# MECLabTUDA/Lifelong-nnUNet

Hardware: AMD Instinct MI355X
Metric: 3D patches/sec (whole node) + mean Dice vs ref, 5-level 3D Generic_UNet training step (higher is better)
Workload: dtype f16 (fp32 accumulate, fp32 master weights); 1 GPU; BASELINE configs[1]: nnUNetTrainerSequential.run_iteration, 160x192x160 patches, batch 2/GPU, num_pool 5, base 32, 3 logits; global_batch=2, parallelism=dp1, distinct_resident_batches=2, deterministic_wgrad=False

## Files before the change

### include/lnn_hip.h

```cpp
#ifndef LNN_HIP_H
#define LNN_HIP_H

#include <stddef.h>
#include <stdint.h>

#ifdef __cplusplus
extern "C" {
#endif

typedef void* lnn_stream_t;

enum lnn_status {
    LNN_OK = 0,
    LNN_ERR_BAD_ARG = -1,
    LNN_ERR_WORKSPACE = -2,
    LNN_ERR_LAUNCH = -3,
    LNN_ERR_UNSUPPORTED = -4
};

const char* lnn_last_error(void);
int lnn_version(void);
int lnn_device_info(int* cu_count, int* clock_khz, char* name, int name_len);

int lnn_pack_weights(lnn_stream_t s, const float* src, void* dst_h, int ntaps, int M, int KC,
// ... 60 lines not shown
int lnn_instnorm_lrelu_seg_bwd(lnn_stream_t s, void* y_inout_h, const void* dz_prior_h, int ld_dz, const float* seg_w,
                               const float* dlogits, float* seg_dw, int K, int N, long V, int C, const float* mean,
                               const float* rstd, const float* gamma, const float* beta, float slope, float* dgamma,
                               float* dbeta, float grad_unscale, double* ws);
size_t lnn_instnorm_lrelu_seg_bwd_ws_doubles(int N, int C);
int lnn_instnorm_lrelu_bwd_sums(lnn_stream_t s, const void* y_h, const void* dz_h, int ld_dz, int N, long V, int C,
                                const float* mean, const float* rstd, const float* gamma, const float* beta, float slope,
                                float* dgamma, float* dbeta, float grad_unscale, double* ws);
int lnn_conv3d_wgrad_c1_in_bwd(lnn_stream_t s, const void* x_h, const void* y_h, const void* dz_h, int ld_dz, float* dwp, int N,
                               int D, int H, int W, int K, const float* mean, const float* rstd, const float* gamma,
                               const float* beta, float slope, const double* ws, float* parts, long parts_elems);
int lnn_conv3d_dgrad_in_bwd_sums(lnn_stream_t s, const void* dy, int ld_dy, const void* wp, void* dx, int ld_dx, int N, int Di,
                                 int Hi, int Wi, int C, int K, const void* u_h, const float* mean, const float* rstd,
                                 const float* gamma, const float* beta, float slope, float* dgamma, float* dbeta,
                                 float grad_unscale, double* ws, float* splitk_ws, long splitk_elems);
int lnn_instnorm_lrelu_bwd_apply(lnn_stream_t s, void* y_h, const void* dz_h, int ld_dz, int N, long V, int C, const float* mean,
                                 const float* rstd, const float* gamma, const float* beta, float slope, double* ws);
int lnn_instnorm_small_volume(void);
int lnn_conv3d_fwd_in_lrelu(lnn_stream_t s, const void* x_a, const void* x_b, int ld_x, int c_a, const void* wp, const float* bias,
                            void* y, int N, int Di, int Hi, int Wi, int C, int K, int stride, float eps, float* mean, float* rstd,
                            const float* gamma, const float* beta, float slope, void* z_h, int ld_z, double* ws, float* splitk_ws,
                            long splitk_elems);
int lnn_conv3d_dgrad_in_bwd(lnn_stream_t s, const void* dy, int ld_dy, const void* wp, void* dx, int ld_dx, int N, int Di, int Hi,
                            int Wi, int C, int K, void* u_h, const float* mean, const float* rstd, const float* gamma,
                            const float* beta, float slope, float* dgamma, float* dbeta, float grad_unscale, double* ws,
                            float* splitk_ws, long splitk_elems);

int lnn_seg1x1_fwd(lnn_stream_t s, const void* z_h, int ld_z, const float* w, float* logits, int N, long V,
                   int C, int K);
int lnn_seg1x1_bwd(lnn_stream_t s, const void* z_h, int ld_z, const float* w, const float* dlogits, void* dz_h,
// ... 117 lines not shown
```

### lifelong-nnunet_amd/csrc/igemm_common.h

```cpp
#pragma once
#include "lnn_common.h"

struct TapTable {
    int ntaps;
    int taps_per_group;
    unsigned short pos_off[27];
    unsigned char slot[27];
};

struct ConvParams {
    const half_t* x;
    const half_t* x2;
    half_t* y2;
    int csplit = 0x7fffffff, msplit = 0x7fffffff;
    const half_t* wp;
    const float* bias;
    half_t* y;
    int ld_x, ld_y;
    int N, Di, Hi, Wi, Do, Ho, Wo;
    int C, M, Mpad, KCpad;
    int wtaps;
    int Ld, Lh, Lw;
    int tiles_z, tiles_y, tiles_x;
    int os, par_z, par_y, par_x;
// ... 28 lines not shown
                            const float* beta, float slope, float* mean, float* rstd);
int lnn_launch_in_small_bwd(hipStream_t s, void* y, const void* dz, int ld_dz, int N, long V, int C, const float* mean, const float* rstd,
                            const float* gamma, const float* beta, float slope, double* ws, float* dgamma, float* dbeta, float unscale);
int lnn_launch_in_stats_finalize(hipStream_t s, const float* pws, int nslots, int N, int C, long V, float eps, float* mean, float* rstd);
int lnn_launch_in_bwd_sums_raw(hipStream_t s, const float* pws, int nslots, int N, int C, const float* mean, const float* rstd,
                               double* ws, float* dgamma, float* dbeta, float unscale);
int lnn_launch_conv_s1_v9(hipStream_t s, ConvParams& p, const char* name);
int lnn_conv_k133_on_v9(hipStream_t s, const void* x, int ld_x, const void* wp, const float* bias, void* y, int ld_y, int N, int D, int H,
                        int W, int C, int M, int flip, const char* name);
bool lnn_conv_s1_mt_supported(const ConvParams& p);
double lnn_conv_s1_mt_efficiency(const ConvParams& p);
int lnn_conv_s1_mt_ksplit(const ConvParams& p, const float* ws, long ws_elems);
int lnn_launch_conv_s1_mt(hipStream_t s, ConvParams& p, float* ws, long ws_elems, const char* name);
int lnn_launch_up2_dgrad(hipStream_t s, ConvParams& p, const char* name);
int lnn_launch_up2_convT(hipStream_t s, ConvParams& p, const char* name);
int lnn_launch_down2_conv(hipStream_t s, ConvParams& p, const char* name);
int lnn_launch_down2_convT_dgrad(hipStream_t s, ConvParams& p, const char* name);
bool lnn_down2s_supported(const ConvParams& p);
int lnn_down2s_stats_slots(const ConvParams& p);
int lnn_launch_down2s(hipStream_t s, ConvParams& p, const char* name);
```

### lifelong-nnunet_amd/csrc/igemm_conv.hip

```cpp
#include "lnn_common.h"
#include "igemm_common.h"
#include "igemm_gen.h"
#include <cstdlib>

namespace {

typedef unsigned c1_uint4 __attribute__((ext_vector_type(4)));

template <bool STATS>
__global__ __launch_bounds__(256, 3) void conv_c1_fwd_kernel(const ConvParams p, int tiles_per_sample) {
    constexpr int TZ = 4, TY = 8, TX = 8, VT = TZ * TY * TX / 128, PZ = TZ + 2, PY = TY + 2, PX = TX + 2, P = PZ * PY * PX;
    constexpr int NL = (P + 255) / 256;
    __shared__ half_t xl[P];
    __shared__ float sred[STATS ? 4 * 2 * 32 : 1];
    const int tid = threadIdx.x, lane = tid & 63, wave = tid >> 6;
    const int n = blockIdx.y;
    const int m0 = blockIdx.z * 32;
    const long xbase_n = (long)n * p.Di * p.Hi * p.Wi;
    const int v = lane & 31, hk = lane >> 5;
    half8 a[2];
#pragma unroll
    for (int k16 = 0; k16 < 2; ++k16) a[k16] = *reinterpret_cast<const half8*>(p.wp + lnn_panel_off(0, m0 + v, k16 * 16 + hk * 8, 1, 32));
    int toff[2][8];
#pragma unroll
// ... 373 lines not shown
}
}

extern "C" int lnn_conv3d_dgrad(lnn_stream_t s, const void* dy, int ld_dy, const void* wp, void* dx, int ld_dx, int N,
                                int Di, int Hi, int Wi, int C, int K, int stride, int accumulate) {
    return conv3d_dgrad_impl(s, dy, ld_dy, wp, dx, nullptr, 0, ld_dx, N, Di, Hi, Wi, C, K, stride, accumulate);
}

extern "C" int lnn_conv3d_dgrad_ws(lnn_stream_t s, const void* dy, int ld_dy, const void* wp, void* dx, int ld_dx, int N, int Di, int Hi,
                                   int Wi, int C, int K, int stride, int accumulate, float* splitk_ws, long splitk_elems) {
    return conv3d_dgrad_impl(s, dy, ld_dy, wp, dx, nullptr, 0, ld_dx, N, Di, Hi, Wi, C, K, stride, accumulate, splitk_ws, splitk_elems);
}

static int g_last_dgrad_reduce_fused = 0;
extern "C" int lnn_debug_last_dgrad_reduce_fused(void) { return g_last_dgrad_reduce_fused; }

extern "C" int lnn_conv3d_dgrad_in_bwd_sums(lnn_stream_t s_, const void* dy, int ld_dy, const void* wp, void* dx, int ld_dx, int N,
                                            int Di, int Hi, int Wi, int C, int K, const void* u, const float* mean, const float* rstd,
                                            const float* gamma, const float* beta, float slope, float* dgamma, float* dbeta,
                                            float grad_unscale, double* ws, float* splitk_ws, long splitk_elems) {
    hipStream_t s = (hipStream_t)s_;
    LNN_REQUIRE(u && lnn_aligned16(u) && mean && rstd && gamma && beta && ws, "lnn_conv3d_dgrad_in_bwd_sums: null / misaligned parameter");
    const long V = (long)Di * Hi * Wi;
    ConvParams p{};
    p.x = (const half_t*)dy; p.y = (half_t*)dx; p.ld_x = ld_dy; p.ld_y = ld_dx; p.N = N;
    p.Di = Di; p.Hi = Hi; p.Wi = Wi; p.Do = Di; p.Ho = Hi; p.Wo = Wi; p.C = K; p.M = C; p.os = 1;
    p.Ld = Di; p.Lh = Hi; p.Lw = Wi; p.pad_lo = 1;
    p.red_ld = C;
    static int no_fuse = -1;
    if (no_fuse < 0) { const char* e = getenv("LNN_NO_FUSED_IN_BWD_REDUCE"); no_fuse = (e && e[0] == '1') ? 1 : 0; }
    const bool fused = !no_fuse && wp && dx && dy && lnn_aligned16(dx) && lnn_aligned16(dy) && use_v9(p) && lnn_conv_s1_v9_red_supported(p) &&
                       !lnn_gen_prefers(LNN_GEN_OP_CONV_S1, (long)N * V);
    g_last_dgrad_reduce_fused = fused ? 1 : 0;
    if (!fused) {
        if (int e = conv3d_dgrad_impl(s_, dy, ld_dy, wp, dx, nullptr, 0, ld_dx, N, Di, Hi, Wi, C, K, 1, 0, splitk_ws, splitk_elems)) return e;
        return lnn_instnorm_lrelu_bwd_sums(s_, u, dx, ld_dx, N, V, C, mean, rstd, gamma, beta, slope, dgamma, dbeta, grad_unscale, ws);
    }
    LNN_REQUIRE(lnn_aligned16(wp), "lnn_conv3d_dgrad_in_bwd_sums: weight panel misaligned");
    if (int e = check_act(dy, ld_dy, K, "lnn_conv3d_dgrad_in_bwd_sums(dy)")) return e;
    if (int e = check_act(dx, ld_dx, C, "lnn_conv3d_dgrad_in_bwd_sums(dx)")) return e;
    p.wp = (const half_t*)wp; p.bias = nullptr;
    p.Mpad = lnn_round_up(C, 32); p.KCpad = lnn_round_up(K, 16); p.wtaps = 27;
    p.taps.ntaps = 27;
    for (int t = 0; t < 27; ++t) {
        const int dz = t / 9, dyy = (t / 3) % 3, dxx = t % 3;
        p.taps.pos_off[t] = (unsigned short)((dz * 10 + dyy) * 10 + dxx);
        p.taps.slot[t] = (unsigned char)((2 - dz) * 9 + (2 - dyy) * 3 + (2 - dxx));
    }
    p.dbg = g_dbg;
    float* pws = reinterpret_cast<float*>(ws + (size_t)N * C * 3);
    p.stats_pws = pws;
    p.red_u = (const half_t*)u; p.red_mean = mean; p.red_rstd = rstd; p.red_gamma = gamma; p.red_beta = beta; p.red_slope = slope;
    if (int e = lnn_launch_conv_s1_v9(s, p, "lnn_conv3d_dgrad_in_bwd_sums(s1,v9,reduce)")) return e;
    return lnn_launch_in_bwd_sums_raw(s, pws, p.stats_nblk, N, C, mean, rstd, ws, dgamma, dbeta, grad_unscale);
}

extern "C" int lnn_conv3d_dgrad_in_bwd(lnn_stream_t s_, const void* dy, int ld_dy, const void* wp, void* dx, int ld_dx, int N, int Di,
                                       int Hi, int Wi, int C, int K, void* u, const float* mean, const float* rstd, const float* gamma,
                                       const float* beta, float slope, float* dgamma, float* dbeta, float grad_unscale, double* ws,
                                       float* splitk_ws, long splitk_elems) {
    LNN_REQUIRE(u && lnn_aligned16(u) && mean && rstd && gamma && beta && ws, "lnn_conv3d_dgrad_in_bwd: null / misaligned parameter");
    const long V = (long)Di * Hi * Wi;
    LNN_REQUIRE(V <= lnn_instnorm_small_volume(), "lnn_conv3d_dgrad_in_bwd: %ld voxels per sample (limit %d): use lnn_conv3d_dgrad_in_bwd_sums",
                V, lnn_instnorm_small_volume());
    LNN_REQUIRE(C % 8 == 0, "lnn_conv3d_dgrad_in_bwd: %d channels (multiple of 8)", C);
    if (int rc = conv3d_dgrad_impl(s_, dy, ld_dy, wp, dx, nullptr, 0, ld_dx, N, Di, Hi, Wi, C, K, 1, 0, splitk_ws, splitk_elems)) return rc;
    return lnn_launch_in_small_bwd((hipStream_t)s_, u, dx, ld_dx, N, V, C, mean, rstd, gamma, beta, slope, ws, dgamma, dbeta, grad_unscale);
}

// ... 74 lines not shown
```

### lifelong-nnunet_amd/csrc/igemm_up2.hip

```cpp
#include "igemm_common.h"

namespace {

constexpr int TZ = 2, TY = 8, TX = 8, PZ = 3, PY = 9, PX = 9;
constexpr int P = PZ * PY * PX;
constexpr int CK = 16, ROWB = 32, MB = 32;
constexpr int XBYTES = P * ROWB;
constexpr int XCHUNKS = P * 2;
constexpr int NT = 256;
constexpr int XN = (XCHUNKS + NT - 1) / NT;

template <int MODE>
struct UpCfg {
    static constexpr int NTAP = MODE == 0 ? 27 : 8;
    static constexpr int WBYTES = NTAP * MB * ROWB;
    static constexpr int WCHUNKS = NTAP * MB * 2;
    static constexpr int WN = (WCHUNKS + NT - 1) / NT;
};

__device__ __forceinline__ int up_xaddr(int pz, int py, int px, int c2) {
    return ((pz * PY + py) * PX + px) * ROWB + ((c2 ^ (py & 1)) << 4);
}
__device__ __forceinline__ int up_waddr(int row, int c2) { return row * ROWB + ((c2 ^ ((row >> 3) & 1)) << 4); }

__device__ __forceinline__ void up_lane_voxel(int v, int& r, int& x) {
    if (v < 4) { r = 0; x = v; }
    else if (v < 12) { r = 2; x = v - 4; }
    else if (v < 16) { r = 0; x = v - 8; }
    else if (v < 20) { r = 3; x = v - 16; }
    else if (v < 28) { r = 1; x = v - 20; }
    else { r = 3; x = v - 24; }
}

template <int MODE>
__global__ __launch_bounds__(NT, 2) void igemm_up2_kernel(const ConvParams p, int mblocks) {
    using Cfg = UpCfg<MODE>;
    constexpr int WN = Cfg::WN, WBYTES = Cfg::WBYTES, WCHUNKS = Cfg::WCHUNKS;
    extern __shared__ __attribute__((aligned(16))) char smem[];
    char* const xb = smem;
    char* const wb = smem + 2 * XBYTES;

    const int tid = threadIdx.x, lane = tid & 63, wave = tid >> 6;
    const int v = lane & 31, hk = lane >> 5;
    const int m0 = (blockIdx.x % mblocks) * MB;
    int t = blockIdx.x / mblocks;
    const int tx = t % p.tiles_x; t /= p.tiles_x;
    const int ty = t % p.tiles_y; t /= p.tiles_y;
    const int tz = t % p.tiles_z; t /= p.tiles_z;
    const int n = t, qz0 = tz * TZ, qy0 = ty * TY, qx0 = tx * TX;
    const int nchunks = (p.C + CK - 1) / CK;
// ... 128 lines not shown
        __syncthreads();
    }

    constexpr int RS = 1040;
    char* const stg = smem;
    const int qz = qz0 + wz, qy = qy0 + wy;
    const int skey = (vx >> 1) & 3;
    const int eox = (lane >> 2) & 15, ec = lane & 3;
    const int egx = 2 * qx0 + eox, em = m0 + ec * 8;
    auto out_ptr = [&](int pz, int rr) -> half8* {
        const int row = wave * 8 + rr, zl = row >> 4, oyl = row & 15;
        const int oz = 2 * (qz0 + zl) + pz, oy = 2 * qy0 + oyl;
        const bool ok = oz < p.Do && oy < p.Ho && egx < p.Wo && em < p.M;
        return ok ? reinterpret_cast<half8*>(p.y + ((((long)n * p.Do + oz) * p.Ho + oy) * p.Wo + egx) * p.ld_y + em) : nullptr;
    };
#pragma unroll
    for (int pz = 0; pz < 2; ++pz) {
        half8 olds[8];
        if (p.accumulate) {
#pragma unroll
            for (int rr = 0; rr < 8; ++rr) {
                const half8* d = out_ptr(pz, rr);
                olds[rr] = *(d ? d : reinterpret_cast<const half8*>(p.y));
            }
        }
#pragma unroll
        for (int c4 = 0; c4 < 4; ++c4) {
            const int cls = pz * 4 + c4, py = c4 >> 1, px = c4 & 1;
            char* vb = stg + (wz * 16 + 2 * wy + py) * RS + (2 * vx + px) * 64;
#pragma unroll
            for (int qq = 0; qq < 4; ++qq) {
                const half4 o = {(half_t)acc[cls][qq * 4 + 0], (half_t)acc[cls][qq * 4 + 1], (half_t)acc[cls][qq * 4 + 2],
                                 (half_t)acc[cls][qq * 4 + 3]};
                *reinterpret_cast<half4*>(vb + (((2 * qq + hk) ^ skey) << 3)) = o;
            }
        }
        __syncthreads();
        {
            const int rkey = (eox >> 2) & 3;
#pragma unroll
            for (int rr = 0; rr < 8; ++rr) {
                const int row = wave * 8 + rr;
                half8 v = *reinterpret_cast<const half8*>(stg + row * RS + eox * 64 + ((ec ^ (rkey >> 1)) << 4));
                if (rkey & 1) v = half8{v[4], v[5], v[6], v[7], v[0], v[1], v[2], v[3]};
                half8* dst = out_ptr(pz, rr);
                if (dst) {
                    if (p.accumulate) {
#pragma unroll
                        for (int e = 0; e < 8; ++e) v[e] = (half_t)((float)v[e] + (float)olds[rr][e]);
                    }
                    *dst = v;
                }
            }
        }
        if (pz == 0) __syncthreads();
    }
    (void)qz; (void)qy;
}

template <int MODE>
int launch_up2(hipStream_t s, ConvParams& p, const char* name) {
    using Cfg = UpCfg<MODE>;
    p.tiles_z = lnn_cdiv((p.Do + 1) / 2, TZ); p.tiles_y = lnn_cdiv((p.Ho + 1) / 2, TY); p.tiles_x = lnn_cdiv((p.Wo + 1) / 2, TX);
    const int mblocks = lnn_cdiv(p.M, MB);
    const long blocks = (long)p.N * p.tiles_z * p.tiles_y * p.tiles_x * mblocks;
    const size_t lds_main = 2 * XBYTES + 2 * Cfg::WBYTES, lds_stage = 32 * 1040;
    const size_t lds = lds_main > lds_stage ? lds_main : lds_stage;
    auto kern = igemm_up2_kernel<MODE>;
    static bool attr_set = false;
    if (!attr_set) {
        hipFuncSetAttribute(reinterpret_cast<const void*>(kern), hipFuncAttributeMaxDynamicSharedMemorySize, 80 * 1024);
        attr_set = true;
    }
    hipLaunchKernelGGL(kern, dim3((unsigned)blocks), dim3(NT), lds, s, p, mblocks);
    LNN_CHECK_LAUNCH(name);
    return LNN_OK;
}

}

int lnn_launch_up2_dgrad(hipStream_t s, ConvParams& p, const char* name) { return launch_up2<0>(s, p, name); }
int lnn_launch_up2_convT(hipStream_t s, ConvParams& p, const char* name) { return launch_up2<1>(s, p, name); }
```

### lifelong-nnunet_amd/csrc/norm_act.hip

```cpp
#include "igemm_common.h"

namespace {

constexpr int NT = 256;
typedef float float2v __attribute__((ext_vector_type(2)));
constexpr int MAX_BLOCKS = 1024;
constexpr int UNR = 4;

__device__ __forceinline__ half8 ld8(const half_t* p, int nt) {
    return nt ? __builtin_nontemporal_load(reinterpret_cast<const half8*>(p)) : *reinterpret_cast<const half8*>(p);
}
__device__ __forceinline__ void st8(half_t* p, const half8& v, int nt) {
    if (nt) __builtin_nontemporal_store(v, reinterpret_cast<half8*>(p));
    else *reinterpret_cast<half8*>(p) = v;
}
int in_nt_flag() {
    static int v = -1;
    if (v < 0) { const char* e = getenv("LNN_IN_NT"); v = (e && e[0] == '1') ? 1 : 0; }
    return v;
}

struct RowMap {
    int C8, VPB, c8, vl;
    bool active;
// ... 307 lines not shown
            for (int u = 0; u < U2; ++u) {
                x[u] = *reinterpret_cast<const half8*>(yp + (v + u * step) * C);
                d[u] = *reinterpret_cast<const half8*>(dp + (v + u * step) * ld_dz);
            }
#pragma unroll
            for (int u = 0; u < U2; ++u) accum(x[u], d[u]);
        }
        for (; v < end; v += step)
            accum(*reinterpret_cast<const half8*>(yp + v * C), *reinterpret_cast<const half8*>(dp + v * ld_dz));
    }
    block_channel_reduce<2>(rm, C, part, red, [&](int a, int c, float s) {
        pws[(((long)a * gridDim.x + blockIdx.x) * gridDim.y + n) * C + c] = s;
    });
}

__device__ __forceinline__ void in_bwd_sums_block(const float* pws, int nblk, int N, int C, int blk, double* red, double* ws,
                                                  float* dgamma, float* dbeta, float unscale, const float* raw_mean = nullptr,
                                                  const float* raw_rstd = nullptr) {
    const int ii = threadIdx.x % FEB, sl = threadIdx.x / FEB;
    const int c = blk * FEB + ii, NC = N * C;
    double g0 = 0, g1 = 0;
    for (int n = 0; n < N; n += 2) {
        const bool two = n + 1 < N;
        double o[4] = {0, 0, 0, 0};
        if (c < C) {
            const float* p0 = pws + n * C + c;
            o[0] = slice_sum<FSL>(p0, NC, nblk, sl);
            o[1] = slice_sum<FSL>(p0 + (long)nblk * NC, NC, nblk, sl);
            if (two) {
                o[2] = slice_sum<FSL>(p0 + C, NC, nblk, sl);
                o[3] = slice_sum<FSL>(p0 + C + (long)nblk * NC, NC, nblk, sl);
            }
        }
        reduce_slices<FSL, 4>(o, red);
        if (c < C && sl == 0) {
            const long i0 = (long)n * C + c;
            if (raw_mean) {
                o[1] = (double)raw_rstd[i0] * (o[1] - (double)raw_mean[i0] * o[0]);
                if (two) o[3] = (double)raw_rstd[i0 + C] * (o[3] - (double)raw_mean[i0 + C] * o[2]);
            }
            ws[i0 * 3 + 0] = o[0]; ws[i0 * 3 + 1] = o[1];
            g0 += o[0]; g1 += o[1];
            if (two) {
                ws[(i0 + C) * 3 + 0] = o[2]; ws[(i0 + C) * 3 + 1] = o[3];
                g0 += o[2]; g1 += o[3];
            }
        }
    }
    if (c >= C || sl != 0) return;
    if (dgamma) atomicAdd(dgamma + c, (float)(g1 * unscale));
    if (dbeta) atomicAdd(dbeta + c, (float)(g0 * unscale));
}
__global__ void in_lrelu_bwd_sums_kernel(const float* pws, int nblk, int NC, int C, double* ws, float* dgamma, float* dbeta,
                                         float unscale, const float* raw_mean, const float* raw_rstd) {
    __shared__ double red[4 * 256];
    in_bwd_sums_block(pws, nblk, NC / C, C, blockIdx.x, red, ws, dgamma, dbeta, unscale, raw_mean, raw_rstd);
}

template <bool DBIAS>
__global__ __launch_bounds__(NT) void in_lrelu_bwd_apply_kernel(half_t* __restrict__ y, const half_t* __restrict__ dz, int ld_dz,
                                                                long V, int C, const float* __restrict__ mean,
                                                                const float* __restrict__ rstd, const float* __restrict__ gamma,
                                                                const float* __restrict__ beta, float slope, const double* ws,
                                                                float* pws, int nt) {
    __shared__ float red[NT * 9];
    const RowMap rm = row_map(C);
    const int n = blockIdx.y;
    float part[1][8];
#pragma unroll
    for (int e = 0; e < 8; ++e) part[0][e] = 0.f;
    if (rm.active) {
// ... 522 lines not shown
    LNN_REQUIRE(V <= SMALL_V, "lnn_instnorm_lrelu_bwd(small): %ld voxels per sample exceed the single-launch limit %d", V, SMALL_V);
    hipLaunchKernelGGL(in_small_bwd_kernel, dim3(lnn_cdiv(C, 32)), dim3(SNT), 0, s, (half_t*)y, (const half_t*)dz, ld_dz, N, (int)V, C, mean,
                       rstd, gamma, beta, slope, ws, dgamma, dbeta, unscale);
    LNN_CHECK_LAUNCH("lnn_instnorm_lrelu_bwd(small)");
    return LNN_OK;
}

int lnn_launch_in_stats_finalize(hipStream_t s, const float* pws, int nslots, int N, int C, long V, float eps, float* mean, float* rstd) {
    hipLaunchKernelGGL(in_stats_finalize_kernel, dim3(lnn_cdiv(N * C, FEB)), dim3(256), 0, s, pws, nslots, N * C, V, eps, mean, rstd);
    LNN_CHECK_LAUNCH("lnn_instnorm_stats(finalize, fused partials)");
    return LNN_OK;
}

int lnn_launch_in_bwd_sums_raw(hipStream_t s, const float* pws, int nslots, int N, int C, const float* mean, const float* rstd,
                               double* ws, float* dgamma, float* dbeta, float unscale) {
    hipLaunchKernelGGL(in_lrelu_bwd_sums_kernel, dim3(lnn_cdiv(C, FEB)), dim3(256), 0, s, pws, nslots, N * C, C, ws, dgamma, dbeta,
                       unscale, mean, rstd);
    LNN_CHECK_LAUNCH("lnn_conv3d_dgrad_in_bwd_sums(sums)");
    return LNN_OK;
}

extern "C" size_t lnn_instnorm_ws_doubles(int N, int C) { return (size_t)N * C * 3 + (size_t)MAX_BLOCKS * N * C; }

extern "C" int lnn_instnorm_stats(lnn_stream_t s_, const void* y, int N, long V, int C, float eps, float* mean, float* rstd,
                                  double* ws) {
    hipStream_t s = (hipStream_t)s_;
    if (int e = check_common(y, N, V, C, "lnn_instnorm_stats")) return e;
    LNN_REQUIRE(mean && rstd && ws, "lnn_instnorm_stats: null output/workspace");
    float* pws = reinterpret_cast<float*>(ws + (size_t)N * C * 3);
    const int nblk = blocks_for(V, C);
    hipLaunchKernelGGL(in_stats_kernel, dim3(nblk, N), dim3(NT), 0, s, (const half_t*)y, V, C, pws);
    LNN_CHECK_LAUNCH("lnn_instnorm_stats");
// ... 150 lines not shown
```

### lifelong-nnunet_amd/engine.py

```python
from __future__ import annotations

from dataclasses import dataclass, field
from typing import List, Optional

import os

import torch

from . import native as nat

LRELU_SLOPE = 1e-2
IN_EPS = 1e-5


class Act:

    def __init__(self, buf: torch.Tensor, off: int, C: int):
        self.buf, self.off, self.C = buf, off, C
        self.ld = buf.shape[-1]
        self.N = buf.shape[0]
        self.dims = tuple(buf.shape[1:4])
        self.V = self.dims[0] * self.dims[1] * self.dims[2]

    def data_ptr(self):
# ... 34 lines not shown
    gx2: Optional[Act] = None
    y: Optional[torch.Tensor] = None
    z: Optional[Act] = None
    gz: Optional[Act] = None
    mean: Optional[torch.Tensor] = None
    rstd: Optional[torch.Tensor] = None
    w: ParamSlot = None
    b: ParamSlot = None
    gamma: ParamSlot = None
    beta: ParamSlot = None
    wp_fwd: int = 0
    wp_dgrad: int = 0
    panel: int = 0
    in_dims: tuple = ()
    x_block: object = None
    wgrad_333: bool = False

    @property
    def iso(self):
        return self.stride != 0

    @property
    def ntaps(self):
        return self.kernel[0] * self.kernel[1] * self.kernel[2]


@dataclass
class UpBlock:
    prefix: str
    cin: int
# ... 166 lines not shown
        x, gx = (None, None) if self.c1_path else (Act(self.image, 0, self.cin_pad), None)
        cin = in_channels
        for d in range(num_pool):
            u = num_pool - 1 - d
            if self.split_cat[u]:
                skip, gskip = Act(self.cat[u][1], 0, feats[d]), Act(self.gcat[u][1], 0, feats[d])
            else:
                skip = Act(self.cat[u], feats[d], feats[d])
                gskip = Act(self.gcat[u], feats[d], feats[d])
            in_dims = dims[d - 1] if d > 0 else dims[0]
            b0 = new_block(f"conv_blocks_context.{d}.blocks.0", cin, feats[d], pools[d - 1] if d > 0 else one, kernels[d],
                           x, gx, d > 0, None, None, in_dims)
            if d == 0:
                b0.first = True
                b0.cin_k = 1 if self.c1_path else self.cin_pad
            b1 = new_block(f"conv_blocks_context.{d}.blocks.1", feats[d], feats[d], one, kernels[d], b0.z, b0.gz, False,
                           skip, gskip, dims[d])
            b1.x_block = b0
            x, gx, cin = b1.z, b1.gz, feats[d]
        nb = num_pool
        b0 = new_block(f"conv_blocks_context.{nb}.0.blocks.0", cin, feats[nb], pools[nb - 1], kernels[nb], x, gx, True, None, None,
                       dims[nb - 1])
        b1 = new_block(f"conv_blocks_context.{nb}.1.blocks.0", feats[nb], feats[nb], one, kernels[nb], b0.z, b0.gz, False, None, None,
                       dims[nb])
        b1.x_block = b0
        x, gx, cdown = b1.z, b1.gz, feats[nb]
        for u in range(num_pool):
            d = num_pool - 1 - u
            cs = feats[d]
            if self.split_cat[u]:
                up_y, up_gy = Act(self.cat[u][0], 0, cs), Act(self.gcat[u][0], 0, cs)
                cat_act, gcat_act = up_y, up_gy
            else:
                up_y, up_gy = Act(self.cat[u], 0, cs), Act(self.gcat[u], 0, cs)
                cat_act, gcat_act = Act(self.cat[u], 0, 2 * cs), Act(self.gcat[u], 0, 2 * cs)
            up = UpBlock(f"tu.{u}", cdown, cs, strides=pools[-(u + 1)], x=x, gx=gx, y=up_y, gy=up_gy)
            up.w = arena.by_name[f"tu.{u}.weight"]
# ... 91 lines not shown
                return 1
            mp = -(-ch // 32) * 32
            waves = classes * -(-(vox // classes) // 64) * -(-mp // 64)
            ks = 1
            while waves * ks * 2 <= 2048 and ks < 64:
                ks *= 2
            return ks * vox * mp if ks > 1 else 1
        for blk in self.blocks:
            if blk.cin_k == 1:
                continue
            ncls = blk.strides[0] * blk.strides[1] * blk.strides[2]
            need = max(need, gen_need(N * blk.z.V, blk.cout, 1, not blk.iso))
            need = max(need, gen_need(N * blk.in_dims[0] * blk.in_dims[1] * blk.in_dims[2], blk.cin_k, ncls, not blk.iso))
        for up in self.ups:
            need = max(need, gen_need(N * up.y.V, up.cout, up.ntaps, not up.iso), gen_need(N * up.x.V, up.cin, 1, not up.iso, 20000))
        self.splitk_ws = torch.zeros(need, dtype=torch.float32, device=dev)
        self.packed_version = -1
        self.unused_heads: List[str] = []
        self._sides = {}
        self.overlap_wgrad = os.environ.get("LNN_NO_WGRAD_OVERLAP", "0") != "1"
        self.deterministic_wgrad = os.environ.get("LNN_DETERMINISTIC_WGRAD", "0") == "1"
        self._det_buf = None
        self.fuse_seg_fwd = os.environ.get("LNN_NO_FUSED_SEG", "0") != "1"
        self.numeric_conv_bias_grad = os.environ.get("LNN_NUMERIC_CONV_BIAS_GRAD", "0") == "1"
        self.fuse_in_stats = os.environ.get("LNN_NO_FUSED_IN_STATS", "0") != "1"
        self.fuse_seg_bwd = os.environ.get("LNN_NO_FUSED_SEG_BWD", "0") != "1"
        self.fuse_first_bwd = os.environ.get("LNN_NO_FUSED_FIRST_BWD", "0") != "1"
        self.fuse_in_bwd_reduce = os.environ.get("LNN_NO_FUSED_IN_BWD_REDUCE", "0") != "1"
        self.small_v = nat.query("lnn_instnorm_small_volume") if os.environ.get("LNN_IN_SMALL", "1") != "0" else 0
        self.probe = None
# ... 296 lines not shown
                    self._probed("dgrad", item, lambda: nat.call(
                        "lnn_conv3d_dgrad_in_bwd", item.y, K, self._wp(item.wp_dgrad), item.gx, item.gx.ld,
                        N, D, H, W, C, K, xb.y, xb.mean, xb.rstd, self.pview(xb.gamma),
                        self.pview(xb.beta), LRELU_SLOPE, self.pview(xb.gamma, self.grad), self.pview(xb.beta, self.grad), 1.0, ws,
                        splitk_ws, splitk_ws.numel()))
                    normed.add(id(xb))
                elif (self.fuse_in_bwd_reduce and item.x_block is not None and item.stride == 1 and item.gx2 is None
                      and not item.gx_accumulate and not self.numeric_conv_bias_grad):
                    xb = item.x_block
                    self._probed("dgrad", item, lambda: nat.call(
                        "lnn_conv3d_dgrad_in_bwd_sums", item.y, K, self._wp(item.wp_dgrad), item.gx, item.gx.ld,
                        N, D, H, W, C, K, xb.y, xb.mean, xb.rstd, self.pview(xb.gamma),
                        self.pview(xb.beta), LRELU_SLOPE, self.pview(xb.gamma, self.grad), self.pview(xb.beta, self.grad), 1.0, ws,
                        splitk_ws, splitk_ws.numel()))
                    presummed.add(id(xb))
                elif item.gx2 is not None:
                    self._probed("dgrad", item, lambda: nat.call(
                        "lnn_conv3d_dgrad_cat_ws", item.y, K, self._wp(item.wp_dgrad), item.gx,
                        item.gx2, item.gx.ld, item.gx.C, N, D, H, W, C, K, 1 if item.gx_accumulate else 0,
                        splitk_ws, splitk_ws.numel()))
                else:
                    self._probed("dgrad", item, lambda: nat.call(
                        "lnn_conv3d_dgrad_ws", item.y, K, self._wp(item.wp_dgrad), item.gx, item.gx.ld,
                        N, D, H, W, C, K, item.stride, 1 if item.gx_accumulate else 0, splitk_ws,
                        splitk_ws.numel()))
            else:
                D, H, W = item.x.dims
                C, K = item.cin, item.cout

                def up_wgrad(item=item, C=C, K=K, D=D, H=H, W=W):
# ... 69 lines not shown
```

### lifelong-nnunet_amd/native.py

```python
from __future__ import annotations

import ctypes as C
import os

_HERE = os.path.dirname(os.path.abspath(__file__))
LIB_PATH = os.environ.get("LNN_LIB_PATH") or os.path.join(_HERE, "csrc", "liblnn_hip.so")

_p = C.c_void_p
_i = C.c_int
_l = C.c_long
_f = C.c_float
_sz = C.c_size_t

SIGNATURES = {
    "lnn_last_error": (C.c_char_p, []),
    "lnn_version": (_i, []),
    "lnn_device_info": (_i, [C.POINTER(_i), C.POINTER(_i), C.c_char_p, _i]),
    "lnn_pack_weights": (_i, [_p, _p, _p, _i, _i, _i, _l, _l, _l]),
    "lnn_packed_weight_elems": (_sz, [_i, _i, _i]),
    "lnn_conv3d_fwd": (_i, [_p, _p, _i, _p, _p, _p, _i, _i, _i, _i, _i, _i, _i, _i]),
    "lnn_conv3d_dgrad": (_i, [_p, _p, _i, _p, _p, _i, _i, _i, _i, _i, _i, _i, _i, _i]),
    "lnn_conv3d_wgrad": (_i, [_p, _p, _i, _p, _i, _p, _i, _i, _i, _i, _i, _i, _i]),
    "lnn_conv3d_fwd_cat": (_i, [_p, _p, _p, _i, _i, _p, _p, _p, _i, _i, _i, _i, _i, _i, _i]),
    "lnn_conv3d_fwd_in_stats": (_i, [_p, _p, _p, _i, _i, _p, _p, _p, _i, _i, _i, _i, _i, _i, _i, _f, _p, _p, _p, _p, _l]),
# ... 8 lines not shown
    "lnn_conv3d_wgrad_cat_det": (_i, [_p, _p, _p, _i, _i, _p, _i, _p, _i, _i, _i, _i, _i, _i, _p, _l]),
    "lnn_convT3d_k2s2_wgrad_det": (_i, [_p, _p, _i, _p, _i, _p, _i, _i, _i, _i, _i, _i, _p, _l]),
    "lnn_unpack_wgrad": (_i, [_p, _p, _p, _i, _i, _i, _l, _l, _l, _f, _i]),
    "lnn_pack_weights_batched": (_i, [_p, _p, _p, _p, _i, _l]),
    "lnn_unpack_wgrad_batched": (_i, [_p, _p, _p, _p, _i, _l, _f, _i]),
    "lnn_wgrad_panel_elems": (_sz, [_i, _i, _i]),
    "lnn_instnorm_stats": (_i, [_p, _p, _i, _l, _i, _f, _p, _p, _p]),
    "lnn_instnorm_lrelu_fwd": (_i, [_p, _p, _p, _i, _i, _l, _i, _p, _p, _p, _p, _f]),
    "lnn_instnorm_lrelu_seg_fwd": (_i, [_p, _p, _p, _i, _i, _l, _i, _p, _p, _p, _p, _f, _p, _p, _i]),
    "lnn_instnorm_lrelu_bwd": (_i, [_p, _p, _p, _i, _i, _l, _i, _p, _p, _p, _p, _f, _p, _p, _p, _f, _p]),
    "lnn_instnorm_ws_doubles": (_sz, [_i, _i]),
    "lnn_instnorm_lrelu_seg_bwd": (_i, [_p, _p, _p, _i, _p, _p, _p, _i, _i, _l, _i, _p, _p, _p, _p, _f, _p, _p, _f, _p]),
    "lnn_instnorm_lrelu_seg_bwd_ws_doubles": (_sz, [_i, _i]),
    "lnn_instnorm_lrelu_bwd_sums": (_i, [_p, _p, _p, _i, _i, _l, _i, _p, _p, _p, _p, _f, _p, _p, _f, _p]),
    "lnn_conv3d_dgrad_in_bwd_sums": (_i, [_p, _p, _i, _p, _p, _i, _i, _i, _i, _i, _i, _i, _p, _p, _p, _p, _p, _f, _p, _p, _f, _p, _p, _l]),
    "lnn_instnorm_lrelu_bwd_apply": (_i, [_p, _p, _p, _i, _i, _l, _i, _p, _p, _p, _p, _f, _p]),
    "lnn_instnorm_small_volume": (_i, []),
    "lnn_conv3d_fwd_in_lrelu": (_i, [_p, _p, _p, _i, _i, _p, _p, _p, _i, _i, _i, _i, _i, _i, _i, _f, _p, _p, _p, _p, _f, _p, _i, _p, _p, _l]),
    "lnn_conv3d_dgrad_in_bwd": (_i, [_p, _p, _i, _p, _p, _i, _i, _i, _i, _i, _i, _i, _p, _p, _p, _p, _p, _f, _p, _p, _f, _p, _p, _l]),
    "lnn_conv3d_wgrad_c1_in_bwd": (_i, [_p, _p, _p, _p, _i, _p, _i, _i, _i, _i, _i, _p, _p, _p, _p, _f, _p, _p, _l]),
    "lnn_seg1x1_fwd": (_i, [_p, _p, _i, _p, _p, _i, _l, _i, _i]),
    "lnn_seg1x1_bwd": (_i, [_p, _p, _i, _p, _p, _p, _i, _p, _i, _l, _i, _i, _i, _f, _p]),
    "lnn_seg1x1_bwd_ws_floats": (_sz, [_i, _i]),
    "lnn_dice_ce_fwd": (_i, [_p, _p, _p, _i, _i, _l, _i, _f, _p, _p]),
    "lnn_dice_ce_fwd_ds": (_i, [_p, _p, _p, _i, _i, _l, _i, _f, _p, _p, _f, _p, _i]),
    "lnn_dice_ce_bwd": (_i, [_p, _p, _p, _i, _i, _l, _i, _f, _p, _f, _p, _f, _p]),
    "lnn_dice_ce_loss_from_totals": (_i, [_p, _p, _i, _i, _l, _i, _f, _p]),
    "lnn_dice_ce_ws_doubles": (_sz, [_i, _i]),
    "lnn_online_dice_counts": (_i, [_p, _p, _p, _i, _i, _l, _p]),
    "lnn_kl_logits": (_i, [_p, _p, _p, _i, _i, _l, _f, _p, _p]),
# ... 129 lines not shown
```

Before: 103.9 patches/s.

## Fuse instance-norm backward reductions into stride-2 dgrad epilogue

Adds a fused path where the stride-2 (up2) data-gradient conv kernel also computes the per-channel instance-norm/LeakyReLU backward partial sums for the skip block's output. This avoids a separate full pass that re-reads dx and the saved activation to compute dgamma/dbeta sums. Per-tile partials are written to the split-k workspace and reduced by a new wide sums kernel when the slot count is large. The cost is extra register pressure and extra u loads in the dgrad epilogue, plus a larger workspace.

Measured after the change: 104.8 patches/s (median of 6 runs). Within noise of the previous version (+0.9%).

```diff
diff --git a/include/lnn_hip.h b/include/lnn_hip.h
--- a/include/lnn_hip.h
+++ b/include/lnn_hip.h
@@ -98,6 +98,10 @@
                                  int Hi, int Wi, int C, int K, const void* u_h, const float* mean, const float* rstd,
                                  const float* gamma, const float* beta, float slope, float* dgamma, float* dbeta,
                                  float grad_unscale, double* ws, float* splitk_ws, long splitk_elems);
+int lnn_conv3d_dgrad_s2_in_bwd_sums(lnn_stream_t s, const void* dy, int ld_dy, const void* wp, void* dx, int ld_dx, int N, int Di,
+                                    int Hi, int Wi, int C, int K, const void* u_h, const float* mean, const float* rstd,
+                                    const float* gamma, const float* beta, float slope, float* dgamma, float* dbeta,
+                                    float grad_unscale, double* ws, float* splitk_ws, long splitk_elems, int accumulate);
 int lnn_instnorm_lrelu_bwd_apply(lnn_stream_t s, void* y_h, const void* dz_h, int ld_dz, int N, long V, int C, const float* mean,
                                  const float* rstd, const float* gamma, const float* beta, float slope, double* ws);
 int lnn_instnorm_small_volume(void);
diff --git a/lifelong-nnunet_amd/csrc/igemm_common.h b/lifelong-nnunet_amd/csrc/igemm_common.h
--- a/lifelong-nnunet_amd/csrc/igemm_common.h
+++ b/lifelong-nnunet_amd/csrc/igemm_common.h
@@ -66,6 +66,8 @@
 int lnn_launch_conv_s1_mt(hipStream_t s, ConvParams& p, float* ws, long ws_elems, const char* name);
 int lnn_launch_up2_dgrad(hipStream_t s, ConvParams& p, const char* name);
 int lnn_launch_up2_convT(hipStream_t s, ConvParams& p, const char* name);
+long lnn_up2_dgrad_red_elems(const ConvParams& p);
+int lnn_launch_up2_dgrad_red(hipStream_t s, ConvParams& p, const char* name);
 int lnn_launch_down2_conv(hipStream_t s, ConvParams& p, const char* name);
 int lnn_launch_down2_convT_dgrad(hipStream_t s, ConvParams& p, const char* name);
 bool lnn_down2s_supported(const ConvParams& p);
diff --git a/lifelong-nnunet_amd/csrc/igemm_conv.hip b/lifelong-nnunet_amd/csrc/igemm_conv.hip
--- a/lifelong-nnunet_amd/csrc/igemm_conv.hip
+++ b/lifelong-nnunet_amd/csrc/igemm_conv.hip
@@ -411,6 +411,11 @@
 
 static int g_last_dgrad_reduce_fused = 0;
 extern "C" int lnn_debug_last_dgrad_reduce_fused(void) { return g_last_dgrad_reduce_fused; }
+static bool in_bwd_reduce_fusion_off() {
+    static int no_fuse = -1;
+    if (no_fuse < 0) { const char* e = getenv("LNN_NO_FUSED_IN_BWD_REDUCE"); no_fuse = (e && e[0] == '1') ? 1 : 0; }
+    return no_fuse == 1;
+}
 
 extern "C" int lnn_conv3d_dgrad_in_bwd_sums(lnn_stream_t s_, const void* dy, int ld_dy, const void* wp, void* dx, int ld_dx, int N,
                                             int Di, int Hi, int Wi, int C, int K, const void* u, const float* mean, const float* rstd,
@@ -424,9 +429,7 @@
     p.Di = Di; p.Hi = Hi; p.Wi = Wi; p.Do = Di; p.Ho = Hi; p.Wo = Wi; p.C = K; p.M = C; p.os = 1;
     p.Ld = Di; p.Lh = Hi; p.Lw = Wi; p.pad_lo = 1;
     p.red_ld = C;
-    static int no_fuse = -1;
-    if (no_fuse < 0) { const char* e = getenv("LNN_NO_FUSED_IN_BWD_REDUCE"); no_fuse = (e && e[0] == '1') ? 1 : 0; }
-    const bool fused = !no_fuse && wp && dx && dy && lnn_aligned16(dx) && lnn_aligned16(dy) && use_v9(p) && lnn_conv_s1_v9_red_supported(p) &&
+    const bool fused = !in_bwd_reduce_fusion_off() && wp && dx && dy && lnn_aligned16(dx) && lnn_aligned16(dy) && use_v9(p) && lnn_conv_s1_v9_red_supported(p) &&
                        !lnn_gen_prefers(LNN_GEN_OP_CONV_S1, (long)N * V);
     g_last_dgrad_reduce_fused = fused ? 1 : 0;
     if (!fused) {
@@ -450,6 +453,36 @@
     p.red_u = (const half_t*)u; p.red_mean = mean; p.red_rstd = rstd; p.red_gamma = gamma; p.red_beta = beta; p.red_slope = slope;
     if (int e = lnn_launch_conv_s1_v9(s, p, "lnn_conv3d_dgrad_in_bwd_sums(s1,v9,reduce)")) return e;
     return lnn_launch_in_bwd_sums_raw(s, pws, p.stats_nblk, N, C, mean, rstd, ws, dgamma, dbeta, grad_unscale);
+}
+
+extern "C" int lnn_conv3d_dgrad_s2_in_bwd_sums(lnn_stream_t s_, const void* dy, int ld_dy, const void* wp, void* dx, int ld_dx, int N,
+                                               int Di, int Hi, int Wi, int C, int K, const void* u, const float* mean, const float* rstd,
+                                               const float* gamma, const float* beta, float slope, float* dgamma, float* dbeta,
+                                               float grad_unscale, double* ws, float* splitk_ws, long splitk_elems, int accumulate) {
+    hipStream_t s = (hipStream_t)s_;
+    LNN_REQUIRE(u && lnn_aligned16(u) && mean && rstd && gamma && beta && ws, "lnn_conv3d_dgrad_s2_in_bwd_sums: null / misaligned parameter");
+    const long V = (long)Di * Hi * Wi;
+    ConvParams p{};
+    p.x = (const half_t*)dy; p.wp = (const half_t*)wp; p.bias = nullptr; p.y = (half_t*)dx;
+    p.ld_x = ld_dy; p.ld_y = ld_dx; p.N = N;
+    p.Di = (Di - 1) / 2 + 1; p.Hi = (Hi - 1) / 2 + 1; p.Wi = (Wi - 1) / 2 + 1; p.Do = Di; p.Ho = Hi; p.Wo = Wi;
+    p.C = K; p.M = C; p.Mpad = lnn_round_up(C, 32); p.KCpad = lnn_round_up(K, 16); p.wtaps = 27;
+    p.accumulate = accumulate;
+    const bool fused = !in_bwd_reduce_fusion_off() && wp && dx && dy && N > 0 && Di > 0 && Hi > 0 && Wi > 0 && C > 0 && C % 32 == 0 &&
+                       !lnn_gen_prefers(LNN_GEN_OP_CONV_S2, (long)N * V) && splitk_ws && splitk_elems >= lnn_up2_dgrad_red_elems(p);
+    g_last_dgrad_reduce_fused = fused ? 1 : 0;
+    if (!fused) {
+        if (int e = conv3d_dgrad_impl(s_, dy, ld_dy, wp, dx, nullptr, 0, ld_dx, N, Di, Hi, Wi, C, K, 2, accumulate, splitk_ws, splitk_elems))
+            return e;
+        return lnn_instnorm_lrelu_bwd_sums(s_, u, dx, ld_dx, N, V, C, mean, rstd, gamma, beta, slope, dgamma, dbeta, grad_unscale, ws);
+    }
+    LNN_REQUIRE(lnn_aligned16(wp), "lnn_conv3d_dgrad_s2_in_bwd_sums: weight panel misaligned");
+    if (int e = check_act(dy, ld_dy, K, "lnn_conv3d_dgrad_s2_in_bwd_sums(dy)")) return e;
+    if (int e = check_act(dx, ld_dx, C, "lnn_conv3d_dgrad_s2_in_bwd_sums(dx)")) return e;
+    p.stats_pws = splitk_ws;
+    p.red_u = (const half_t*)u; p.red_ld = C; p.red_mean = mean; p.red_rstd = rstd; p.red_gamma = gamma; p.red_beta = beta; p.red_slope = slope;
+    if (int e = lnn_launch_up2_dgrad_red(s, p, "lnn_conv3d_dgrad_s2_in_bwd_sums(s2,up2,reduce)")) return e;
+    return lnn_launch_in_bwd_sums_raw(s, splitk_ws, p.stats_nblk, N, C, mean, rstd, ws, dgamma, dbeta, grad_unscale);
 }
 
 extern "C" int lnn_conv3d_dgrad_in_bwd(lnn_stream_t s_, const void* dy, int ld_dy, const void* wp, void* dx, int ld_dx, int N, int Di,
diff --git a/lifelong-nnunet_amd/csrc/igemm_up2.hip b/lifelong-nnunet_amd/csrc/igemm_up2.hip
--- a/lifelong-nnunet_amd/csrc/igemm_up2.hip
+++ b/lifelong-nnunet_amd/csrc/igemm_up2.hip
@@ -32,8 +32,9 @@
     else { r = 3; x = v - 24; }
 }
 
-template <int MODE>
+template <int MODE, bool RED = false>
 __global__ __launch_bounds__(NT, 2) void igemm_up2_kernel(const ConvParams p, int mblocks) {
+    static_assert(!RED || MODE == 0, "the fused reduce exists for the data gradient only");
     using Cfg = UpCfg<MODE>;
     constexpr int WN = Cfg::WN, WBYTES = Cfg::WBYTES, WCHUNKS = Cfg::WCHUNKS;
     extern __shared__ __attribute__((aligned(16))) char smem[];
@@ -192,6 +193,22 @@
         const bool ok = oz < p.Do && oy < p.Ho && egx < p.Wo && em < p.M;
         return ok ? reinterpret_cast<half8*>(p.y + ((((long)n * p.Do + oz) * p.Ho + oy) * p.Wo + egx) * p.ld_y + em) : nullptr;
     };
+    auto u_ptr = [&](int pz, int rr) -> const half8* {
+        const int row = wave * 8 + rr, zl = row >> 4, oyl = row & 15;
+        const int oz = 2 * (qz0 + zl) + pz, oy = 2 * qy0 + oyl;
+        const bool ok = oz < p.Do && oy < p.Ho && egx < p.Wo && em < p.M;
+        return reinterpret_cast<const half8*>(ok ? p.red_u + ((((long)n * p.Do + oz) * p.Ho + oy) * p.Wo + egx) * p.red_ld + em : p.red_u);
+    };
+    float ra[RED ? 8 : 1], rb[RED ? 8 : 1], rs1[RED ? 8 : 1], rs2[RED ? 8 : 1];
+    if constexpr (RED) {
+#pragma unroll
+        for (int e = 0; e < 8; ++e) {
+            const int c = min(em + e, p.M - 1);
+            ra[e] = p.red_gamma[c] * p.red_rstd[n * p.M + c];
+            rb[e] = p.red_beta[c] - ra[e] * p.red_mean[n * p.M + c];
+            rs1[e] = rs2[e] = 0.f;
+        }
+    }
 #pragma unroll
     for (int pz = 0; pz < 2; ++pz) {
         half8 olds[8];
@@ -212,6 +229,11 @@
                                  (half_t)acc[cls][qq * 4 + 3]};
                 *reinterpret_cast<half4*>(vb + (((2 * qq + hk) ^ skey) << 3)) = o;
             }
+        }
+        half8 us[RED ? 8 : 1];
+        if constexpr (RED) {
+#pragma unroll
+            for (int rr = 0; rr < 8; ++rr) us[rr] = *u_ptr(pz, rr);
         }
         __syncthreads();
         {
@@ -228,26 +250,72 @@
                         for (int e = 0; e < 8; ++e) v[e] = (half_t)((float)v[e] + (float)olds[rr][e]);
                     }
                     *dst = v;
+                    if constexpr (RED) {
+#pragma unroll
+                        for (int e = 0; e < 8; ++e) {
+                            const float dzf = (float)v[e], uf = (float)us[rr][e];
+                            const float pre = __builtin_fmaf(ra[e], uf, rb[e]);
+                            const float g = pre > 0.f ? dzf : dzf * p.red_slope;
+                            rs1[e] += g;
+                            rs2[e] = __builtin_fmaf(g, uf, rs2[e]);
+                        }
+                    }
                 }
             }
         }
         if (pz == 0) __syncthreads();
     }
+    if constexpr (RED) {
+#pragma unroll
+        for (int e = 0; e < 8; ++e) {
+#pragma unroll
+            for (int m = 4; m < 64; m <<= 1) {
+                rs1[e] += __shfl_xor(rs1[e], m);
+                rs2[e] += __shfl_xor(rs2[e], m);
+            }
+        }
+        float* const rl = reinterpret_cast<float*>(smem + 32 * RS);
+        if (lane < 4) {
+#pragma unroll
+            for (int e = 0; e < 8; ++e) {
+                rl[(wave * 2 + 0) * MB + lane * 8 + e] = rs1[e];
+                rl[(wave * 2 + 1) * MB + lane * 8 + e] = rs2[e];
+            }
+        }
+        __syncthreads();
+        if (wave == 0) {
+            const int a = lane >> 5, c = lane & 31;
+            const float tot = ((rl[(0 * 2 + a) * MB + c] + rl[(1 * 2 + a) * MB + c]) + rl[(2 * 2 + a) * MB + c]) + rl[(3 * 2 + a) * MB + c];
+            const int tile = (int)(blockIdx.x / mblocks) - n * p.stats_nblk;
+            if (m0 + c < p.M) p.stats_pws[(((long)a * p.stats_nblk + tile) * p.N + n) * p.M + m0 + c] = tot;
+        }
+    }
     (void)qz; (void)qy;
 }
 
-template <int MODE>
+void up2_tiles(ConvParams& p) {
+    p.tiles_z = lnn_cdiv((p.Do + 1) / 2, TZ); p.tiles_y = lnn_cdiv((p.Ho + 1) / 2, TY); p.tiles_x = lnn_cdiv((p.Wo + 1) / 2, TX);
+}
+
+template <int MODE, bool RED = false>
 int launch_up2(hipStream_t s, ConvParams& p, const char* name) {
     using Cfg = UpCfg<MODE>;
-    p.tiles_z = lnn_cdiv((p.Do + 1) / 2, TZ); p.tiles_y = lnn_cdiv((p.Ho + 1) / 2, TY); p.tiles_x = lnn_cdiv((p.Wo + 1) / 2, TX);
+    up2_tiles(p);
     const int mblocks = lnn_cdiv(p.M, MB);
     const long blocks = (long)p.N * p.tiles_z * p.tiles_y * p.tiles_x * mblocks;
     const size_t lds_main = 2 * XBYTES + 2 * Cfg::WBYTES, lds_stage = 32 * 1040;
     const size_t lds = lds_main > lds_stage ? lds_main : lds_stage;
-    auto kern = igemm_up2_kernel<MODE>;
+    static_assert(!RED || 2 * XBYTES + 2 * Cfg::WBYTES >= 32 * 1040 + 4 * 2 * MB * sizeof(float), "the wave sums sit behind the staging rows");
+    if (RED) {
+        LNN_REQUIRE(p.red_u && p.stats_pws && p.red_mean && p.red_rstd && p.red_gamma && p.red_beta, "%s: null reduce parameter", name);
+        LNN_REQUIRE(p.M % MB == 0 && p.red_ld >= p.M && p.red_ld % 8 == 0, "%s: %d channels / ld %d: no fused-reduce instance", name, p.M, p.red_ld);
+        p.stats_nblk = p.tiles_z * p.tiles_y * p.tiles_x;
+    }
+    auto kern = igemm_up2_kernel<MODE, RED>;
     static bool attr_set = false;
     if (!attr_set) {
-        hipFuncSetAttribute(reinterpret_cast<const void*>(kern), hipFuncAttributeMaxDynamicSharedMemorySize, 80 * 1024);
+        const hipError_t e = hipFuncSetAttribute(reinterpret_cast<const void*>(kern), hipFuncAttributeMaxDynamicSharedMemorySize, 80 * 1024);
+        LNN_REQUIRE(e == hipSuccess, "%s: hipFuncSetAttribute(dynamic LDS): %s", name, hipGetErrorString(e));
         attr_set = true;
     }
     hipLaunchKernelGGL(kern, dim3((unsigned)blocks), dim3(NT), lds, s, p, mblocks);
@@ -259,3 +327,9 @@
 
 int lnn_launch_up2_dgrad(hipStream_t s, ConvParams& p, const char* name) { return launch_up2<0>(s, p, name); }
 int lnn_launch_up2_convT(hipStream_t s, ConvParams& p, const char* name) { return launch_up2<1>(s, p, name); }
+long lnn_up2_dgrad_red_elems(const ConvParams& p) {
+    ConvParams q = p;
+    up2_tiles(q);
+    return 2L * q.tiles_z * q.tiles_y * q.tiles_x * q.N * q.M;
+}
+int lnn_launch_up2_dgrad_red(hipStream_t s, ConvParams& p, const char* name) { return launch_up2<0, true>(s, p, name); }
diff --git a/lifelong-nnunet_amd/csrc/norm_act.hip b/lifelong-nnunet_amd/csrc/norm_act.hip
--- a/lifelong-nnunet_amd/csrc/norm_act.hip
+++ b/lifelong-nnunet_amd/csrc/norm_act.hip
@@ -345,25 +345,27 @@
     });
 }
 
+template <int SL = FSL>
 __device__ __forceinline__ void in_bwd_sums_block(const float* pws, int nblk, int N, int C, int blk, double* red, double* ws,
                                                   float* dgamma, float* dbeta, float unscale, const float* raw_mean = nullptr,
                                                   const float* raw_rstd = nullptr) {
-    const int ii = threadIdx.x % FEB, sl = threadIdx.x / FEB;
-    const int c = blk * FEB + ii, NC = N * C;
+    constexpr int EB = 256 / SL;
+    const int ii = threadIdx.x % EB, sl = threadIdx.x / EB;
+    const int c = blk * EB + ii, NC = N * C;
     double g0 = 0, g1 = 0;
     for (int n = 0; n < N; n += 2) {
         const bool two = n + 1 < N;
         double o[4] = {0, 0, 0, 0};
         if (c < C) {
             const float* p0 = pws + n * C + c;
-            o[0] = slice_sum<FSL>(p0, NC, nblk, sl);
-            o[1] = slice_sum<FSL>(p0 + (long)nblk * NC, NC, nblk, sl);
+            o[0] = slice_sum<SL>(p0, NC, nblk, sl);
+            o[1] = slice_sum<SL>(p0 + (long)nblk * NC, NC, nblk, sl);
             if (two) {
-                o[2] = slice_sum<FSL>(p0 + C, NC, nblk, sl);
-                o[3] = slice_sum<FSL>(p0 + C + (long)nblk * NC, NC, nblk, sl);
-            }
-        }
-        reduce_slices<FSL, 4>(o, red);
+                o[2] = slice_sum<SL>(p0 + C, NC, nblk, sl);
+                o[3] = slice_sum<SL>(p0 + C + (long)nblk * NC, NC, nblk, sl);
+            }
+        }
+        reduce_slices<SL, 4>(o, red);
         if (c < C && sl == 0) {
             const long i0 = (long)n * C + c;
             if (raw_mean) {
@@ -386,6 +388,11 @@
                                          float unscale, const float* raw_mean, const float* raw_rstd) {
     __shared__ double red[4 * 256];
     in_bwd_sums_block(pws, nblk, NC / C, C, blockIdx.x, red, ws, dgamma, dbeta, unscale, raw_mean, raw_rstd);
+}
+__global__ void in_lrelu_bwd_sums_wide_kernel(const float* pws, int nblk, int NC, int C, double* ws, float* dgamma, float* dbeta,
+                                              float unscale, const float* raw_mean, const float* raw_rstd) {
+    __shared__ double red[4 * 256];
+    in_bwd_sums_block<256>(pws, nblk, NC / C, C, blockIdx.x, red, ws, dgamma, dbeta, unscale, raw_mean, raw_rstd);
 }
 
 template <bool DBIAS>
@@ -938,8 +945,12 @@
 
 int lnn_launch_in_bwd_sums_raw(hipStream_t s, const float* pws, int nslots, int N, int C, const float* mean, const float* rstd,
                                double* ws, float* dgamma, float* dbeta, float unscale) {
-    hipLaunchKernelGGL(in_lrelu_bwd_sums_kernel, dim3(lnn_cdiv(C, FEB)), dim3(256), 0, s, pws, nslots, N * C, C, ws, dgamma, dbeta,
-                       unscale, mean, rstd);
+    if (nslots > MAX_BLOCKS)
+        hipLaunchKernelGGL(in_lrelu_bwd_sums_wide_kernel, dim3(C), dim3(256), 0, s, pws, nslots, N * C, C, ws, dgamma, dbeta, unscale, mean,
+                           rstd);
+    else
+        hipLaunchKernelGGL(in_lrelu_bwd_sums_kernel, dim3(lnn_cdiv(C, FEB)), dim3(256), 0, s, pws, nslots, N * C, C, ws, dgamma, dbeta,
+                           unscale, mean, rstd);
     LNN_CHECK_LAUNCH("lnn_conv3d_dgrad_in_bwd_sums(sums)");
     return LNN_OK;
 }
diff --git a/lifelong-nnunet_amd/engine.py b/lifelong-nnunet_amd/engine.py
--- a/lifelong-nnunet_amd/engine.py
+++ b/lifelong-nnunet_amd/engine.py
@@ -72,6 +72,7 @@
     panel: int = 0
     in_dims: tuple = ()
     x_block: object = None
+    x_skip_block: object = None
     wgrad_333: bool = False
 
     @property
@@ -268,6 +269,8 @@
             if d == 0:
                 b0.first = True
                 b0.cin_k = 1 if self.c1_path else self.cin_pad
+            else:
+                b0.x_skip_block = b1
             b1 = new_block(f"conv_blocks_context.{d}.blocks.1", feats[d], feats[d], one, kernels[d], b0.z, b0.gz, False,
                            skip, gskip, dims[d])
             b1.x_block = b0
@@ -275,6 +278,7 @@
         nb = num_pool
         b0 = new_block(f"conv_blocks_context.{nb}.0.blocks.0", cin, feats[nb], pools[nb - 1], kernels[nb], x, gx, True, None, None,
                        dims[nb - 1])
+        b0.x_skip_block = b1
         b1 = new_block(f"conv_blocks_context.{nb}.1.blocks.0", feats[nb], feats[nb], one, kernels[nb], b0.z, b0.gz, False, None, None,
                        dims[nb])
         b1.x_block = b0
@@ -396,6 +400,10 @@
             need = max(need, gen_need(N * blk.in_dims[0] * blk.in_dims[1] * blk.in_dims[2], blk.cin_k, ncls, not blk.iso))
         for up in self.ups:
             need = max(need, gen_need(N * up.y.V, up.cout, up.ntaps, not up.iso), gen_need(N * up.x.V, up.cin, 1, not up.iso, 20000))
+        for blk in self.blocks:
+            if blk.iso and blk.stride == 2 and blk.x_skip_block is not None:
+                od = blk.in_dims
+                need = max(need, 2 * -(-(-(-od[0] // 2)) // 2) * -(-(-(-od[1] // 2)) // 8) * -(-(-(-od[2] // 2)) // 8) * N * blk.cin_k)
         self.splitk_ws = torch.zeros(need, dtype=torch.float32, device=dev)
         self.packed_version = -1
         self.unused_heads: List[str] = []
@@ -722,6 +730,15 @@
                         self.pview(xb.beta), LRELU_SLOPE, self.pview(xb.gamma, self.grad), self.pview(xb.beta, self.grad), 1.0, ws,
                         splitk_ws, splitk_ws.numel()))
                     presummed.add(id(xb))
+                elif (self.fuse_in_bwd_reduce and item.x_skip_block is not None and item.stride == 2 and item.iso and item.gx2 is None
+                      and not self.numeric_conv_bias_grad and item.x_skip_block.z.V > self.small_v):
+                    xb = item.x_skip_block
+                    self._probed("dgrad", item, lambda: nat.call(
+                        "lnn_conv3d_dgrad_s2_in_bwd_sums", item.y, K, self._wp(item.wp_dgrad), item.gx, item.gx.ld,
+                        N, D, H, W, C, K, xb.y, xb.mean, xb.rstd, self.pview(xb.gamma),
+                        self.pview(xb.beta), LRELU_SLOPE, self.pview(xb.gamma, self.grad), self.pview(xb.beta, self.grad), 1.0, ws,
+                        splitk_ws, splitk_ws.numel(), 1 if item.gx_accumulate else 0))
+                    presummed.add(id(xb))
                 elif item.gx2 is not None:
                     self._probed("dgrad", item, lambda: nat.call(
                         "lnn_conv3d_dgrad_cat_ws", item.y, K, self._wp(item.wp_dgrad), item.gx,
diff --git a/lifelong-nnunet_amd/native.py b/lifelong-nnunet_amd/native.py
--- a/lifelong-nnunet_amd/native.py
+++ b/lifelong-nnunet_amd/native.py
@@ -46,6 +46,8 @@
     "lnn_instnorm_lrelu_seg_bwd_ws_doubles": (_sz, [_i, _i]),
     "lnn_instnorm_lrelu_bwd_sums": (_i, [_p, _p, _p, _i, _i, _l, _i, _p, _p, _p, _p, _f, _p, _p, _f, _p]),
     "lnn_conv3d_dgrad_in_bwd_sums": (_i, [_p, _p, _i, _p, _p, _i, _i, _i, _i, _i, _i, _i, _p, _p, _p, _p, _p, _f, _p, _p, _f, _p, _p, _l]),
+    "lnn_conv3d_dgrad_s2_in_bwd_sums": (_i, [_p, _p, _i, _p, _p, _i, _i, _i, _i, _i, _i, _i, _p, _p, _p, _p, _p, _f, _p, _p, _f, _p, _p, _l,
+                                             _i]),
     "lnn_instnorm_lrelu_bwd_apply": (_i, [_p, _p, _p, _i, _i, _l, _i, _p, _p, _p, _p, _f, _p]),
     "lnn_instnorm_small_volume": (_i, []),
     "lnn_conv3d_fwd_in_lrelu": (_i, [_p, _p, _p, _i, _i, _p, _p, _p, _i, _i, _i, _i, _i, _i, _i, _f, _p, _p, _p, _p, _f, _p, _i, _p, _p, _l]),
```
